# cg-tuwien/ppsurf

Measured on AMD Instinct MI355X. Metric: occupancy query-points/sec @ res=257, 50NN, higher is better.
Workload: dtype f16x3

## Files before the change

### ppsurf_amd/csrc/pps_decode.hip

```cpp
#include <cstdlib>
#include "pps_common.h"
#include "../../include/ppsurf_amd.h"

using namespace pps;

#ifndef NT
#define NT 256
#endif
#define NW (NT / 64)
#ifndef WG_PER_CU
#define WG_PER_CU (512 / NT)
#endif
#ifndef PPS_PRIO
#define PPS_PRIO 1
#endif
#ifndef PPS_PRIO_PN
#define PPS_PRIO_PN 1
#endif
#define CH4 2048

template <int CHUNK_F4_NEXT, int NTH = NT, class F>
__device__ __forceinline__ void stream_step(const f32x4* __restrict__ gnext, f32x4*& cur, f32x4*& nxt, F&& compute) {
    chunk_copy_async<CHUNK_F4_NEXT / NTH, NTH>(gnext, nxt);
    compute((const f32x4*)cur);
// ... 579 lines not shown
#pragma unroll
    for (int h = 0; h < PN_C2N; ++h)
        stream_step<PCH4, PNT>(wg + 2048 + (h + 1) * PCH4, cur, nxt, [&](const f32x4* w) {
            dense_blocks_f16x3<2, PN_C2OB, 1>(a, (const half8*)w, bias4 + 48 + 4 * PN_C2OB * h, lane,
                                              [&](int i, const f32x4& o0, const f32x4& o1) { y[PN_C2OB / 2 * h + i] = split_f16_r(amax, o0, o1); }); });
#pragma unroll
    for (int c = 0; c < PN_C3N - 1; ++c)
        stream_step<PCH4, PNT>(wg + 4096 + (c + 1) * PCH4, cur, nxt, [&](const f32x4* w) {
            dense_blocks_f16x3<4, PN_C3OB, 1>(y, (const half8*)w, bias4 + 80 + 4 * PN_C3OB * c, lane,
                                              [&](int i, const f32x4& o0, const f32x4& o1) { z[PN_C3OB * c + 2 * i] = o0; z[PN_C3OB * c + 2 * i + 1] = o1; }); });
    stream_step<1024, PNT>(wg, cur, nxt, [&](const f32x4* w) {
        dense_blocks_f16x3<4, PN_C3OB, 1>(y, (const half8*)w, bias4 + 80 + 4 * PN_C3OB * (PN_C3N - 1), lane,
                                          [&](int i, const f32x4& o0, const f32x4& o1) { z[PN_C3OB * (PN_C3N - 1) + 2 * i] = o0; z[PN_C3OB * (PN_C3N - 1) + 2 * i + 1] = o1; }); });
    __builtin_amdgcn_s_setprio(0);
}

template <int T, class ZSink>
__device__ __forceinline__ void stn_chain_h_tiles(const float (&coord)[T], const float* xyz_l, const f32x4* bias4, const f32x4* wg,
                                                  f32x4*& cur, f32x4*& nxt, int lane, float& amax, ZSink&& zsink) {
    const int g = lane >> 4;
    HiLo a[T][2], b[T][2], y[T][4];
#pragma unroll
    for (int t = 0; t < T; ++t) {
        f32x4 x0[4];
#pragma unroll
        for (int bb = 0; bb < 4; ++bb) x0[bb] = bias4[4 * bb + g];
        xyz_blocks<4>(coord[t], x0, xyz_l, lane);
        relu_blocks<4>(x0);
        a[t][0] = split_f16_r(amax, x0[0], x0[1]);
        a[t][1] = split_f16_r(amax, x0[2], x0[3]);
    }
    __builtin_amdgcn_s_setprio(PPS_PRIO_PN);
    stream_step<1024, PNT>(wg + 1024, cur, nxt, [&](const f32x4* w) {
        dense_blocks_f16x3_tiles<T, 2, 4, 1>(a, (const half8*)w, bias4 + 16, lane, [&](int t, int i, const f32x4& o0, const f32x4& o1) { b[t][i] = split_f16_r(amax, o0, o1); }); });
    stream_step<PCH4, PNT>(wg + 2048, cur, nxt, [&](const f32x4* w) {
        dense_blocks_f16x3_tiles<T, 2, 4, 1>(b, (const half8*)w, bias4 + 32, lane, [&](int t, int i, const f32x4& o0, const f32x4& o1) { a[t][i] = split_f16_r(amax, o0, o1); }); });
#pragma unroll
    for (int h = 0; h < PN_C2N; ++h)
        stream_step<PCH4, PNT>(wg + 2048 + (h + 1) * PCH4, cur, nxt, [&](const f32x4* w) {
            dense_blocks_f16x3_tiles<T, 2, PN_C2OB, 1>(a, (const half8*)w, bias4 + 48 + 4 * PN_C2OB * h, lane,
                                                      [&](int t, int i, const f32x4& o0, const f32x4& o1) { y[t][PN_C2OB / 2 * h + i] = split_f16_r(amax, o0, o1); }); });
#pragma unroll
    for (int c = 0; c < PN_C3N - 1; ++c)
        stream_step<PCH4, PNT>(wg + 4096 + (c + 1) * PCH4, cur, nxt, [&](const f32x4* w) {
            dense_blocks_f16x3_tiles<T, 4, PN_C3OB, 1>(y, (const half8*)w, bias4 + 80 + 4 * PN_C3OB * c, lane,
                                                      [&](int t, int i, const f32x4& o0, const f32x4& o1) { zsink(t, PN_C3OB * c + 2 * i, o0, o1); }); });
    stream_step<1024, PNT>(wg, cur, nxt, [&](const f32x4* w) {
        dense_blocks_f16x3_tiles<T, 4, PN_C3OB, 1>(y, (const half8*)w, bias4 + 80 + 4 * PN_C3OB * (PN_C3N - 1), lane,
                                                  [&](int t, int i, const f32x4& o0, const f32x4& o1) { zsink(t, PN_C3OB * (PN_C3N - 1) + 2 * i, o0, o1); }); });
    __builtin_amdgcn_s_setprio(0);
}

template <bool H>
__global__ __launch_bounds__(PNT, 2) void pointnet_stn_rows_kernel(const float* __restrict__ patches, int64_t Q, int P, int pack,
                                                                   const float* __restrict__ wpack, const f32x4* __restrict__ wdense,
                                                                   const float* __restrict__ bias, float* __restrict__ gout, int* __restrict__ flag) {
    if (!H && gate_closed(flag)) return;
    float amax = 0.f;
    f32x4* buf0 = (f32x4*)pps_smem;
    f32x4* buf1 = buf0 + PCH4;
    float* xyz_l = (float*)(buf1 + PCH4);
    float* bias_l = xyz_l + PA_W_XYZ;
    float* park = bias_l + PA_NBIAS;
    const f32x4* bias4 = (const f32x4*)bias_l;
    const f32x4* wg = wdense;
    const int lane = lane_id(), wave = threadIdx.x >> 6, n = lane & 15, g = lane >> 4;
    float* mypark = park + wave * PN_PARK_ROWS * PN_ROWF;

    lds_fill(xyz_l, wpack, PA_W_XYZ);
    lds_fill(bias_l, bias, PA_NBIAS);
    stream_prologue<1024, PNT>(wg, buf0);
    stream_wait();
    __syncthreads();
    f32x4 *cur = buf0, *nxt = buf1;

    const PatchPacking pk = patch_packing(P, pack);
    const int64_t ngroups = (Q + pk.qg - 1) / pk.qg;
    const int ntiles = (int)((ngroups + PNW - 1) / PNW);
    int first, count, stride;
    xcd_tile_range(ntiles, first, count, stride);
    for (int it = 0; it < count; ++it) {
        const int64_t q0 = ((int64_t)(first + it * stride) * PNW + wave) * pk.qg;
        if constexpr (H) {
            if (pk.packed) {
                const int ql = n / pk.lo;
                const int64_t qq = (q0 + ql < Q) ? q0 + ql : Q - 1;
                const float coord[1] = {(g < 3) ? patches[(qq * P + pk.fb * 16 + (n % pk.lo)) * 3 + g] : 0.f};
                stn_chain_h_tiles<1>(coord, xyz_l, bias4, wg, cur, nxt, lane, amax, [&](int, int bb, const f32x4& o0, const f32x4& o1) {
                    f32x4 m0, m1;
#pragma unroll
                    for (int r = 0; r < 4; ++r) { m0[r] = group_max(o0[r], pk.lo); m1[r] = group_max(o1[r], pk.lo); }
                    if ((n % pk.lo) == 0) { ((f32x4*)(mypark + ql * PN_ROWF))[4 * bb + g] = m0; ((f32x4*)(mypark + ql * PN_ROWF))[4 * (bb + 1) + g] = m1; }
                });
            }
            for (int qi = 0; qi < pk.qg; ++qi) {
                const int64_t q = q0 + qi;
                const bool qv = q < Q;
                const int64_t qc = qv ? q : Q - 1;
                f32x4 rmax[16];
#pragma unroll
                for (int bb = 0; bb < 16; ++bb)
                    rmax[bb] = pk.packed ? ((const f32x4*)(mypark + qi * PN_ROWF))[4 * bb + g] : f32x4{-INFINITY, -INFINITY, -INFINITY, -INFINITY};
                auto zmax = [&](int, int bb, const f32x4& o0, const f32x4& o1) {
#pragma unroll
                    for (int r = 0; r < 4; ++r) { rmax[bb][r] = max_raw(rmax[bb][r], o0[r]); rmax[bb + 1][r] = max_raw(rmax[bb + 1][r], o1[r]); }
                };
                auto row_coord = [&](int rb) {
                    const int row = rb * 16 + n;
                    const int rowc = row < P ? row : P - 1;
                    return (g < 3) ? patches[(qc * P + rowc) * 3 + g] : 0.f;
                };
                int rb = 0;
                for (; rb + 1 < pk.fb; rb += 2) {
                    const float coord[2] = {row_coord(rb), row_coord(rb + 1)};
                    stn_chain_h_tiles<2>(coord, xyz_l, bias4, wg, cur, nxt, lane, amax, zmax);
                }
                if (rb < pk.fb) {
                    const float coord[1] = {row_coord(rb)};
                    stn_chain_h_tiles<1>(coord, xyz_l, bias4, wg, cur, nxt, lane, amax, zmax);
                }
#pragma unroll
                for (int bb = 0; bb < 16; ++bb) {
                    float p0 = rmax[bb][0], p1 = rmax[bb][1], p2 = rmax[bb][2], p3 = rmax[bb][3];
                    row16_max4(p0, p1, p2, p3);
                    if (n == 0 && qv) ((f32x4*)(gout + q * 256))[4 * bb + g] = f32x4{p0, p1, p2, p3};
                }
            }
            continue;
        }
        f32x4 z[16];
        if (pk.packed) {
            const int ql = n / pk.lo;
            const int64_t qq = (q0 + ql < Q) ? q0 + ql : Q - 1;
            const float coord = (g < 3) ? patches[(qq * P + pk.fb * 16 + (n % pk.lo)) * 3 + g] : 0.f;
            if (H) stn_chain_h(coord, z, xyz_l, bias4, wg, cur, nxt, lane, amax); else stn_chain(coord, z, xyz_l, bias4, wg, cur, nxt, lane);
#pragma unroll
            for (int bb = 0; bb < 16; ++bb) {
                f32x4 m;
#pragma unroll
                for (int r = 0; r < 4; ++r) m[r] = group_max(z[bb][r], pk.lo);
                if ((n % pk.lo) == 0) ((f32x4*)(mypark + ql * PN_ROWF))[4 * bb + g] = m;
            }
        }
        for (int qi = 0; qi < pk.qg; ++qi) {
            const int64_t q = q0 + qi;
            const bool qv = q < Q;
            const int64_t qc = qv ? q : Q - 1;
            f32x4 rmax[16];
#pragma unroll
            for (int bb = 0; bb < 16; ++bb)
                rmax[bb] = pk.packed ? ((const f32x4*)(mypark + qi * PN_ROWF))[4 * bb + g] : f32x4{-INFINITY, -INFINITY, -INFINITY, -INFINITY};
            for (int rb = 0; rb < pk.fb; ++rb) {
                const int row = rb * 16 + n;
                const int rowc = row < P ? row : P - 1;
                const float coord = (g < 3) ? patches[(qc * P + rowc) * 3 + g] : 0.f;
                if (H) stn_chain_h(coord, z, xyz_l, bias4, wg, cur, nxt, lane, amax); else stn_chain(coord, z, xyz_l, bias4, wg, cur, nxt, lane);
#pragma unroll
                for (int bb = 0; bb < 16; ++bb)
#pragma unroll
                    for (int r = 0; r < 4; ++r) rmax[bb][r] = max_raw(rmax[bb][r], z[bb][r]);
            }
#pragma unroll
            for (int bb = 0; bb < 16; ++bb) {
                float p0 = rmax[bb][0], p1 = rmax[bb][1], p2 = rmax[bb][2], p3 = rmax[bb][3];
                row16_max4(p0, p1, p2, p3);
                const f32x4 p = {p0, p1, p2, p3};
                if (n == 0 && qv) ((f32x4*)(gout + q * 256))[4 * bb + g] = p;
            }
        }
    }
    if (H) range_commit(amax, flag);
}

#define PB_NBIAS (128 + 64 + 4096)
#define PB_LDS_BYTES (2 * CH4 * 16 + 4096 * 4)
#ifndef PB_T
#define PB_T 1
#endif

__global__ __launch_bounds__(NT, 2) void pointnet_stn_fc_kernel(const float* __restrict__ gin, int64_t Q,
                                                                const float* __restrict__ wpack, const float* __restrict__ bias,
                                                                float* __restrict__ trans2, const int* __restrict__ gate) {
    if (gate_closed(gate)) return;
    f32x4* buf0 = (f32x4*)pps_smem;
    f32x4* buf1 = buf0 + CH4;
    float* bias_l = (float*)(buf1 + CH4);
    const f32x4* bias4 = (const f32x4*)bias_l;
    const f32x4* wg = (const f32x4*)wpack;
    const int lane = lane_id(), wave = threadIdx.x >> 6, n = lane & 15, g = lane >> 4;

    lds_fill(bias_l, bias + 192, 4096);
    const f32x4* bias_g = (const f32x4*)bias;
    stream_prologue<CH4>(wg, buf0);
    stream_wait();
    __syncthreads();
    f32x4 *cur = buf0, *nxt = buf1;

    const int ntiles = (int)((Q + NW * 16 * PB_T - 1) / (NW * 16 * PB_T));
    int first, count, stride;
    xcd_tile_range(ntiles, first, count, stride);
    for (int it = 0; it < count; ++it) {
        f32x4 u[PB_T][4];
        int64_t qcs[PB_T];
        bool qvs[PB_T];
#pragma unroll
        for (int t = 0; t < PB_T; ++t) {
            const int64_t qi = (int64_t)(first + it * stride) * (NW * 16 * PB_T) + (wave * PB_T + t) * 16 + n;
            qvs[t] = qi < Q;
            qcs[t] = qvs[t] ? qi : Q - 1;
            f32x4 a[16], h[8];
            {
                const f32x4* src = (const f32x4*)(gin + qcs[t] * 256) + g;
#pragma unroll
                for (int bb = 0; bb < 16; ++bb) a[bb] = src[4 * bb];
            }
#pragma unroll
            for (int c = 0; c < 4; ++c)
                stream_step<CH4>(wg + (c + 1) * CH4, cur, nxt,
                               [&](const f32x4* w) { dense_blocks<16, 2, 1>(a, &h[2 * c], w, bias_g + 8 * c, lane); });
            stream_step<CH4>(t + 1 < PB_T ? wg : wg + 5 * CH4, cur, nxt,
                           [&](const f32x4* w) { dense_blocks<8, 4, 1>(h, u[t], w, bias_g + 32, lane); });
        }
#pragma unroll 1
        for (int c = 0; c < 32; ++c) {
            f32x4 o[PB_T][8];
            const f32x4* gn = (c + 1 < 32) ? wg + (6 + c) * CH4 : wg;
            stream_step<CH4>(gn, cur, nxt, [&](const f32x4* w) {
#pragma unroll
                for (int t = 0; t < PB_T; ++t) dense_blocks<4, 8, 0>(u[t], o[t], w, bias4 + 32 * c, lane);
            });
#pragma unroll
            for (int t = 0; t < PB_T; ++t) {
                if (qvs[t]) {
                    f32x4* dst = (f32x4*)(trans2 + qcs[t] * 4096) + g;
#pragma unroll
                    for (int j = 0; j < 8; ++j) dst[4 * (8 * c + j)] = o[t][j];
                }
            }
        }
    }
}

__global__ __launch_bounds__(NT, 2) void pointnet_stn_fc_h_kernel(const float* __restrict__ gin, int64_t Q, const f32x4* __restrict__ w16,
                                                                  const float* __restrict__ bias, half8* __restrict__ trans2h, int* __restrict__ range) {
    float amax = 0.f;
    f32x4* buf0 = (f32x4*)pps_smem;
    f32x4* buf1 = buf0 + CH4;
    float* bias_l = (float*)(buf1 + CH4);
    const f32x4* bias4 = (const f32x4*)bias_l;
    const f32x4* wg = w16;
    const int lane = lane_id(), wave = threadIdx.x >> 6, n = lane & 15, g = lane >> 4;

    lds_fill(bias_l, bias + 192, 4096);
    const f32x4* bias_g = (const f32x4*)bias;
    stream_prologue<CH4>(wg, buf0);
    stream_wait();
    __syncthreads();
    f32x4 *cur = buf0, *nxt = buf1;
    const int ntiles = (int)((Q + NW * 16 - 1) / (NW * 16));
    int first, count, stride;
    xcd_tile_range(ntiles, first, count, stride);
    for (int it = 0; it < count; ++it) {
        const int64_t qi = (int64_t)(first + it * stride) * (NW * 16) + wave * 16 + n;
        const bool qv = qi < Q;
        const int64_t qc = qv ? qi : Q - 1;
        HiLo ah[8], h[4], u[2];
        {
            f32x4 a[16];
            const f32x4* src = (const f32x4*)(gin + qc * 256) + g;
#pragma unroll
            for (int bb = 0; bb < 16; ++bb) a[bb] = src[4 * bb];
#pragma unroll
            for (int kb = 0; kb < 8; ++kb) ah[kb] = split_f16_r(amax, a[2 * kb], a[2 * kb + 1]);
        }
#pragma unroll
        for (int c = 0; c < 4; ++c)
            stream_step<CH4>(wg + (c + 1) * CH4, cur, nxt, [&](const f32x4* w) {
                dense_blocks_f16x3<8, 2, 1>(ah, (const half8*)w, bias_g + 8 * c, lane, [&](int, const f32x4& o0, const f32x4& o1) { h[c] = split_f16_r(amax, o0, o1); }); });
        stream_step<CH4>(wg + 5 * CH4, cur, nxt, [&](const f32x4* w) {
            dense_blocks_f16x3<4, 4, 1>(h, (const half8*)w, bias_g + 32, lane, [&](int i, const f32x4& o0, const f32x4& o1) { u[i] = split_f16_r(amax, o0, o1); }); });
        half8* dst = trans2h + qc * 1024 + g;
#pragma unroll 1
        for (int c = 0; c < 32; ++c) {
            const f32x4* gn = (c + 1 < 32) ? wg + (6 + c) * CH4 : wg;
            stream_step<CH4>(gn, cur, nxt, [&](const f32x4* w) {
                dense_blocks_f16x3<2, 8, 0, false>(u, (const half8*)w, bias4 + 32 * c, lane, [&](int i, const f32x4& o0, const f32x4& o1) {
                    const int a = 2 * c + (i >> 1), kb = i & 1;
                    const HiLo v = split_f16_r(amax, o0, o1);
                    if (qv) {
                        half8* d = dst + (((a >> 4) * 2 + kb) * 2) * 64 + 4 * (a & 15);
                        d[0] = v.hi;
                        d[64] = v.lo;
                    }
                }); });
        }
    }
    range_commit(amax, range);
}

#define PC_W_XYZ 256
#define PC_NBIAS (576 + 256 + 4)
#define PC_WFLOATS (4096 + 8192)
#define PC_LDS_BYTES ((PC_WFLOATS + PC_W_XYZ + PC_NBIAS) * 4)

template <bool H>
__global__ __launch_bounds__(PNT, 2) void pointnet_feat_rows_kernel(const float* __restrict__ patches, const float* __restrict__ trans2,
                                                                    int64_t Q, int P, const float* __restrict__ wpack,
                                                                    const f32x4* __restrict__ wdense, const float* __restrict__ bias,
                                                                    float* __restrict__ xbar, int* __restrict__ flag) {
    if (!H && gate_closed(flag)) return;
    float amax = 0.f;
    f32x4* w_l = (f32x4*)pps_smem;
    float* xyz_l = (float*)(w_l + PC_WFLOATS / 4);
    float* bias_l = xyz_l + PC_W_XYZ;
    const f32x4* bias4 = (const f32x4*)bias_l;
    const f32x4* u4 = bias4 + 144;
    const int lane = lane_id(), wave = threadIdx.x >> 6, n = lane & 15, g = lane >> 4;
    for (int i = threadIdx.x; i < PC_WFLOATS / 4; i += PNT) w_l[i] = wdense[i];
    lds_fill(xyz_l, wpack, PC_W_XYZ);
    lds_fill(bias_l, bias, PC_NBIAS);
    __syncthreads();
    const float s0 = bias_l[576 + 256];
    const f32x4* w_c0b = w_l;
    const f32x4* w_c2 = w_l + 1024;
    const int ntile_rows = (P + 15) / 16;

    const int ntiles = (int)((Q + PNW - 1) / PNW);
    int first, count, stride;
    xcd_tile_range(ntiles, first, count, stride);
    for (int it = 0; it < count; ++it) {
        const int64_t q = (int64_t)(first + it * stride) * PNW + wave;
        if (q >= Q) continue;
        half8 th[4][2], tl[4][2];
        f32x4 tf[4][4];
        if (H) {
            const half8* tq = (const half8*)trans2 + q * 1024 + 4 * n + g;
#pragma unroll
            for (int ob = 0; ob < 4; ++ob)
#pragma unroll
                for (int kb = 0; kb < 2; ++kb) { th[ob][kb] = tq[((ob * 2 + kb) * 2) * 64]; tl[ob][kb] = tq[((ob * 2 + kb) * 2 + 1) * 64]; }
        } else {
            const f32x4* tq = (const f32x4*)(trans2 + q * 4096);
#pragma unroll
            for (int ob = 0; ob < 4; ++ob)
#pragma unroll
                for (int kb = 0; kb < 4; ++kb) tf[ob][kb] = tq[(16 * ob + n) * 16 + 4 * kb + g];
        }
        f32x4 acc[8];
        float mrun = -INFINITY, ssum = 0.f;
#pragma unroll
        for (int bb = 0; bb < 8; ++bb) acc[bb] = f32x4{0.f, 0.f, 0.f, 0.f};
        for (int rb = 0; rb < ntile_rows; ++rb) {
            const int rowi = rb * 16 + n;
            const bool valid = rowi < P;
            const int rowc = valid ? rowi : P - 1;
            const float coord = (g < 3) ? patches[(q * P + rowc) * 3 + g] : 0.f;
            f32x4 x0[4], y[8];
#pragma unroll
            for (int bb = 0; bb < 4; ++bb) x0[bb] = bias4[4 * bb + g];
            xyz_blocks<4>(coord, x0, xyz_l, lane);
            relu_blocks<4>(x0);
            __builtin_amdgcn_s_setprio(PPS_PRIO_PN);
            float s = 0.f;
            if (H) {
                HiLo a[2], b[2];
                a[0] = split_f16_r(amax, x0[0], x0[1]);
                a[1] = split_f16_r(amax, x0[2], x0[3]);
                dense_blocks_f16x3<2, 4, 1>(a, (const half8*)w_c0b, bias4 + 16, lane, [&](int i, const f32x4& o0, const f32x4& o1) { b[i] = split_f16_r(amax, o0, o1); });
#pragma unroll
                for (int ob = 0; ob < 4; ++ob) {
                    f32x4 o = bias4[32 + 4 * ob + g], c = {0.f, 0.f, 0.f, 0.f};
#pragma unroll
                    for (int kb = 0; kb < 2; ++kb) {
                        o = __builtin_amdgcn_mfma_f32_16x16x32_f16(th[ob][kb], b[kb].hi, o, 0, 0, 0);
                        c = __builtin_amdgcn_mfma_f32_16x16x32_f16(th[ob][kb], b[kb].lo, c, 0, 0, 0);
                        c = __builtin_amdgcn_mfma_f32_16x16x32_f16(tl[ob][kb], b[kb].hi, c, 0, 0, 0);
                    }
                    o += c;
#pragma unroll
                    for (int r = 0; r < 4; ++r) x0[ob][r] = fmaxf(o[r], 0.f);
                }
                a[0] = split_f16_r(amax, x0[0], x0[1]);
                a[1] = split_f16_r(amax, x0[2], x0[3]);
                dense_blocks_f16x3<2, 8, 1>(a, (const half8*)w_c2, bias4 + 48, lane, [&](int i, const f32x4& o0, const f32x4& o1) {
                    const f32x4 w0 = u4[4 * (2 * i) + g], w1 = u4[4 * (2 * i + 1) + g];
#pragma unroll
                    for (int r = 0; r < 4; ++r) s += w0[r] * o0[r] + w1[r] * o1[r];
                    y[2 * i] = o0;
                    y[2 * i + 1] = o1;
                });
            } else {
                f32x4 x1[4];
                dense_blocks<4, 4, 1>(x0, x1, w_c0b, bias4 + 16, lane);
#pragma unroll
                for (int ob = 0; ob < 4; ++ob) {
                    f32x4 o = bias4[32 + 4 * ob + g];
#pragma unroll
                    for (int kb = 0; kb < 4; ++kb) {
                        o = __builtin_amdgcn_mfma_f32_16x16x4f32(tf[ob][kb].x, x1[kb].x, o, 0, 0, 0);
                        o = __builtin_amdgcn_mfma_f32_16x16x4f32(tf[ob][kb].y, x1[kb].y, o, 0, 0, 0);
                        o = __builtin_amdgcn_mfma_f32_16x16x4f32(tf[ob][kb].z, x1[kb].z, o, 0, 0, 0);
                        o = __builtin_amdgcn_mfma_f32_16x16x4f32(tf[ob][kb].w, x1[kb].w, o, 0, 0, 0);
                    }
#pragma unroll
                    for (int r = 0; r < 4; ++r) x0[ob][r] = fmaxf(o[r], 0.f);
                }
                dense_blocks<4, 8, 1>(x0, y, w_c2, bias4 + 48, lane);
#pragma unroll
                for (int bb = 0; bb < 8; ++bb) {
                    const f32x4 w4 = u4[4 * bb + g];
#pragma unroll
                    for (int r = 0; r < 4; ++r) s += w4[r] * y[bb][r];
                }
            }
            __builtin_amdgcn_s_setprio(0);
            s += __shfl_xor(s, 16);
            s += __shfl_xor(s, 32);
            s += s0;
            const float mblk = row16_max(valid ? s : -INFINITY);
            const float mnew = fmaxf(mrun, mblk);
            const float scale = __expf(mrun - mnew);
            const float en = valid ? __expf(s - mnew) : 0.f;
            mrun = mnew;
            ssum = ssum * scale + en;
#pragma unroll
            for (int bb = 0; bb < 8; ++bb)
#pragma unroll
                for (int r = 0; r < 4; ++r) acc[bb][r] = acc[bb][r] * scale + en * y[bb][r];
        }
        const float inv = 1.f / row16_sum(ssum);
        rows16_sum_transposed8(acc, lane);
        if (n < 8) ((f32x4*)(xbar + q * 128))[4 * n + g] = acc[0] * inv;
    }
    if (H) range_commit(amax, flag);
}

#define TL_NBIAS (256 + 256 + 32)
#define TL_LDS_BYTES (2 * CH4 * 16 + TL_NBIAS * 4)

__global__ __launch_bounds__(NT, 2) void decode_tail_kernel(const float* __restrict__ pooled, const float* __restrict__ xbar, int64_t Q,
                                                            const float* __restrict__ wpack, const float* __restrict__ bias,
                                                            float* __restrict__ logits, float* __restrict__ occ, int* __restrict__ gate) {
    if (gate_closed(gate)) return;
    if (gate != nullptr && blockIdx.x == 0 && threadIdx.x == 0) atomicAdd(gate + 1, 1);
    f32x4* buf0 = (f32x4*)pps_smem;
    f32x4* buf1 = buf0 + CH4;
    float* bias_l = (float*)(buf1 + CH4);
    const f32x4* bias4 = (const f32x4*)bias_l;
    const f32x4* wg = (const f32x4*)wpack;
    const int lane = lane_id(), wave = threadIdx.x >> 6, n = lane & 15, g = lane >> 4;

    lds_fill(bias_l, bias, TL_NBIAS);
    stream_prologue<CH4>(wg, buf0);
    stream_wait();
    __syncthreads();
    f32x4 *cur = buf0, *nxt = buf1;

    const int ntiles = (int)((Q + NW * 16 - 1) / (NW * 16));
    int first, count, stride;
    xcd_tile_range(ntiles, first, count, stride);
    for (int it = 0; it < count; ++it) {
        const int64_t qi = (int64_t)(first + it * stride) * (NW * 16) + wave * 16 + n;
        const bool qv = qi < Q;
        const int64_t qc = qv ? qi : Q - 1;
        f32x4 p[16], x[8], h[16];
        {
            const f32x4* sp = (const f32x4*)(pooled + qc * 256) + g;
            const f32x4* sx = (const f32x4*)(xbar + qc * 128) + g;
#pragma unroll
            for (int bb = 0; bb < 16; ++bb) p[bb] = sp[4 * bb];
#pragma unroll
            for (int bb = 0; bb < 8; ++bb) x[bb] = sx[4 * bb];
        }
#pragma unroll
        for (int c = 0; c < 8; ++c)
            stream_step<CH4>(wg + (c + 1) * CH4, cur, nxt,
                           [&](const f32x4* w) { dense_blocks<16, 2, 0>(p, &h[2 * c], w, bias4 + 8 * c, lane); });
#pragma unroll
        for (int c = 0; c < 4; ++c)
            stream_step<CH4>(wg + (c + 9) * CH4, cur, nxt,
                           [&](const f32x4* w) { dense_blocks<8, 4, 1, 1>(x, &h[4 * c], w, bias4, lane); });
#pragma unroll
        for (int c = 0; c < 8; ++c)
            stream_step<CH4>(wg + (c + 13) * CH4, cur, nxt,
                           [&](const f32x4* w) { dense_blocks<16, 2, 1>(h, &p[2 * c], w, bias4 + 64 + 8 * c, lane); });
        f32x4 o[2];
        stream_step<CH4>(wg, cur, nxt, [&](const f32x4* w) { dense_blocks<16, 2, 0>(p, o, w, bias4 + 128, lane); });
        if (qv && g == 0) {
            const float l0 = o[0].x, l1 = o[0].y;
            logits[qi * 2] = l0;
            logits[qi * 2 + 1] = l1;
            if (occ) {
                const float mx = fmaxf(l0, l1);
                const float e0 = __expf(l0 - mx), e1 = __expf(l1 - mx);
                occ[qi] = (e0 - e1) / (e0 + e1);
            }
        }
    }
}

__global__ __launch_bounds__(NT, 2) void decode_tail_h_kernel(const float* __restrict__ pooled, const float* __restrict__ xbar, int64_t Q,
                                                              const f32x4* __restrict__ w16, const float* __restrict__ bias,
                                                              float* __restrict__ logits, float* __restrict__ occ, int* __restrict__ range) {
    float amax = 0.f;
    f32x4* buf0 = (f32x4*)pps_smem;
    f32x4* buf1 = buf0 + CH4;
    float* bias_l = (float*)(buf1 + CH4);
    const f32x4* bias4 = (const f32x4*)bias_l;
    const f32x4* wg = w16;
    const int lane = lane_id(), wave = threadIdx.x >> 6, n = lane & 15, g = lane >> 4;

// ... 6 lines not shown
    const int ntiles = (int)((Q + NW * 16 - 1) / (NW * 16));
    int first, count, stride;
    xcd_tile_range(ntiles, first, count, stride);
    for (int it = 0; it < count; ++it) {
        const int64_t qi = (int64_t)(first + it * stride) * (NW * 16) + wave * 16 + n;
        const bool qv = qi < Q;
        const int64_t qc = qv ? qi : Q - 1;
        HiLo p[8], x[4];
        {
            const f32x4* sp = (const f32x4*)(pooled + qc * 256) + g;
            const f32x4* sx = (const f32x4*)(xbar + qc * 128) + g;
#pragma unroll
            for (int kb = 0; kb < 8; ++kb) p[kb] = split_f16_r(amax, sp[4 * (2 * kb)], sp[4 * (2 * kb + 1)]);
#pragma unroll
            for (int kb = 0; kb < 4; ++kb) x[kb] = split_f16_r(amax, sx[4 * (2 * kb)], sx[4 * (2 * kb + 1)]);
        }
        HiLo y[8];
#pragma unroll
        for (int c = 0; c < 8; ++c) {
            f32x4 h[2];
            stream_step<CH4 / 2>(wg + c * 3072 + 2048, cur, nxt, [&](const f32x4* w) {
                dense_blocks_f16x3<8, 2, 0>(p, (const half8*)w, bias4 + 8 * c, lane, [&](int, const f32x4& o0, const f32x4& o1) { h[0] = o0; h[1] = o1; }); });
            stream_step<CH4>(c + 1 < 8 ? wg + (c + 1) * 3072 : wg + 24576, cur, nxt, [&](const f32x4* w) {
                dense_blocks_f16x3<4, 2, 1, true, true>(x, (const half8*)w, bias4, lane, [&](int, const f32x4& o0, const f32x4& o1) { y[c] = split_f16_r(amax, o0, o1); }, h); });
        }
#pragma unroll
        for (int c = 0; c < 8; ++c)
            stream_step<CH4>(wg + 24576 + (c + 1) * 2048, cur, nxt, [&](const f32x4* w) {
                dense_blocks_f16x3<8, 2, 1>(y, (const half8*)w, bias4 + 64 + 8 * c, lane, [&](int, const f32x4& o0, const f32x4& o1) { p[c] = split_f16_r(amax, o0, o1); }); });
        f32x4 o[2];
        stream_step<CH4>(wg, cur, nxt, [&](const f32x4* w) {
            dense_blocks_f16x3<8, 2, 0>(p, (const half8*)w, bias4 + 128, lane, [&](int, const f32x4& o0, const f32x4& o1) { o[0] = o0; o[1] = o1; }); });
        if (qv && g == 0) {
            const float l0 = o[0].x, l1 = o[0].y;
            logits[qi * 2] = l0;
            logits[qi * 2 + 1] = l1;
            if (occ) {
                const float mx = fmaxf(l0, l1);
                const float e0 = __expf(l0 - mx), e1 = __expf(l1 - mx);
                occ[qi] = (e0 - e1) / (e0 + e1);
            }
        }
    }
    range_commit(amax, range);
}

static int g_cu_count = 0;
static int cu_count() {
    if (g_cu_count == 0) {
        int dev = 0;
        hipDeviceProp_t prop;
        if (hipGetDevice(&dev) != hipSuccess || hipGetDeviceProperties(&prop, dev) != hipSuccess) return -1;
        g_cu_count = prop.multiProcessorCount;
    }
    return g_cu_count;
}

template <class K>
static int set_lds(K kernel, int bytes) {
    return hipFuncSetAttribute((const void*)kernel, hipFuncAttributeMaxDynamicSharedMemorySize, bytes) == hipSuccess ? 0 : 1;
}

static int grid_for(int64_t ntiles) {
    int cus = cu_count();
    if (cus <= 0) cus = 256;
    cus *= WG_PER_CU;
    return (int)(ntiles < cus ? (ntiles > 0 ? ntiles : 1) : cus);
}

struct PnSplit { int64_t q_packed; int grid_packed, grid_rest, rest_mode; };
static PnSplit pn_split(int64_t q, int p) {
    int cus = cu_count();
    if (cus <= 0) cus = 256;
    const PatchPacking pk = patch_packing(p);
    PnSplit sp;
    const int wgs = cus * PN_WG_PER_CU;
    const int64_t per_round = (int64_t)wgs * PNW * pk.qg;
    sp.q_packed = pk.packed ? (q / per_round) * per_round : 0;
    if (pk.packed && getenv("PPS_PN_FORCE_PACK")) sp.q_packed = q;
    sp.grid_packed = wgs;
    sp.rest_mode = pk.packed ? 2 : 0;
    const int64_t rest_tiles = (q - sp.q_packed + PNW - 1) / PNW;
    sp.grid_rest = (int)(rest_tiles < wgs ? rest_tiles : wgs);
    return sp;
}

#define PPS_LAUNCH_CHECK() (hipGetLastError() == hipSuccess ? PPS_OK : PPS_ERR_LAUNCH)

template <bool H>
static int launch_stn_rows(const float* patches, int64_t q, int p, const float* wpack, const void* wdense, const float* bias, float* g,
                           int* flag, void* stream) {
    static int once = set_lds(pointnet_stn_rows_kernel<H>, PA_LDS_BYTES);
    (void)once;
    const PnSplit sp = pn_split(q, p);
    if (sp.q_packed > 0)
        hipLaunchKernelGGL(pointnet_stn_rows_kernel<H>, dim3(sp.grid_packed), dim3(PNT), PA_LDS_BYTES, (hipStream_t)stream, patches,
                           sp.q_packed, p, 1, wpack, (const f32x4*)wdense, bias, g, flag);
    if (q > sp.q_packed)
        hipLaunchKernelGGL(pointnet_stn_rows_kernel<H>, dim3(sp.grid_rest), dim3(PNT), PA_LDS_BYTES, (hipStream_t)stream,
                           patches + sp.q_packed * p * 3, q - sp.q_packed, p, sp.rest_mode, wpack, (const f32x4*)wdense, bias, g + sp.q_packed * 256, flag);
    return PPS_LAUNCH_CHECK();
}

template <bool H>
static int launch_feat_rows(const float* patches, const float* trans2, int64_t q, int p, const float* wpack, const void* wdense,
                            const float* bias, float* xbar, int* flag, void* stream) {
    static int once = set_lds(pointnet_feat_rows_kernel<H>, PC_LDS_BYTES);
    (void)once;
    int cus = cu_count();
    if (cus <= 0) cus = 256;
    const int64_t ntiles = (q + PNW - 1) / PNW, wgs = (int64_t)cus * PN_WG_PER_CU;
    hipLaunchKernelGGL(pointnet_feat_rows_kernel<H>, dim3((unsigned)(ntiles < wgs ? ntiles : wgs)), dim3(PNT), PC_LDS_BYTES, (hipStream_t)stream, patches,
                       trans2, q, p, wpack, (const f32x4*)wdense, bias, xbar, flag);
    return PPS_LAUNCH_CHECK();
}


static int interp_pool_f32_impl(const float* G, const float* pts, const float* query, const int64_t* idx, int64_t q, int k,
                                const float* wpack, const float* bias, float* pooled, const int* gate, void* stream) {
    if (q < 0 || k < 1 || k > 64) return PPS_ERR_ARG;
    if (q == 0) return PPS_OK;
    if (!G || !pts || !query || !idx || !wpack || !bias || !pooled) return PPS_ERR_ARG;
    static int once = set_lds(interp_pool_kernel, IP_LDS_BYTES);
    (void)once;
    hipLaunchKernelGGL(interp_pool_kernel, dim3(grid_for((q + NW / 4 - 1) / (NW / 4))), dim3(NT), IP_LDS_BYTES, (hipStream_t)stream,
                       G, pts, query, idx, q, k, wpack, bias, pooled, gate);
    return PPS_LAUNCH_CHECK();
}

static int stn_fc_f32_impl(const float* g, int64_t q, const float* wpack, const float* bias, float* trans2, const int* gate, void* stream) {
    if (q < 0) return PPS_ERR_ARG;
    if (q == 0) return PPS_OK;
    if (!g || !wpack || !bias || !trans2) return PPS_ERR_ARG;
    static int once = set_lds(pointnet_stn_fc_kernel, PB_LDS_BYTES);
    (void)once;
    hipLaunchKernelGGL(pointnet_stn_fc_kernel, dim3(grid_for((q + NW * 16 * PB_T - 1) / (NW * 16 * PB_T))), dim3(NT), PB_LDS_BYTES, (hipStream_t)stream,
                       g, q, wpack, bias, trans2, gate);
    return PPS_LAUNCH_CHECK();
}

static int decode_tail_f32_impl(const float* pooled, const float* xbar, int64_t q, const float* wpack, const float* bias,
                                float* logits, float* occ, int* gate, void* stream) {
    if (q < 0) return PPS_ERR_ARG;
    if (q == 0) return PPS_OK;
    if (!pooled || !xbar || !wpack || !bias || !logits) return PPS_ERR_ARG;
    static int once = set_lds(decode_tail_kernel, TL_LDS_BYTES);
    (void)once;
    hipLaunchKernelGGL(decode_tail_kernel, dim3(grid_for((q + NW * 16 - 1) / (NW * 16))), dim3(NT), TL_LDS_BYTES, (hipStream_t)stream,
                       pooled, xbar, q, wpack, bias, logits, occ, gate);
    return PPS_LAUNCH_CHECK();
}

extern "C" {

int pps_abi_version(void) { return 2; }

int pps_debug_occupancy(int which) {
    int n = -1;
    if (which == 0) { set_lds(interp_pool_kernel, IP_LDS_BYTES); hipOccupancyMaxActiveBlocksPerMultiprocessor(&n, interp_pool_kernel, NT, IP_LDS_BYTES); }
    if (which == 1) { set_lds(pointnet_stn_rows_kernel<false>, PA_LDS_BYTES); hipOccupancyMaxActiveBlocksPerMultiprocessor(&n, pointnet_stn_rows_kernel<false>, PNT, PA_LDS_BYTES); }
    if (which == 3) { set_lds(pointnet_stn_fc_kernel, PB_LDS_BYTES); hipOccupancyMaxActiveBlocksPerMultiprocessor(&n, pointnet_stn_fc_kernel, NT, PB_LDS_BYTES); }
    if (which == 4) { set_lds(pointnet_stn_fc_h_kernel, PB_LDS_BYTES); hipOccupancyMaxActiveBlocksPerMultiprocessor(&n, pointnet_stn_fc_h_kernel, NT, PB_LDS_BYTES); }
    if (which == 2) { set_lds(pointnet_feat_rows_kernel<false>, PC_LDS_BYTES); hipOccupancyMaxActiveBlocksPerMultiprocessor(&n, pointnet_feat_rows_kernel<false>, PNT, PC_LDS_BYTES); }
    return n;
}
int pps_device_cu_count(void) { return cu_count(); }
// ... 27 lines not shown
    if (cus <= 0) cus = 256;
    const int64_t ntiles = (q + IH_NW / 4 - 1) / (IH_NW / 4);
    const int64_t wgs = (int64_t)cus * IH_WG_PER_CU;
    const int grid = (int)(ntiles < wgs ? ntiles : wgs);
    hipLaunchKernelGGL(interp_pool_f16x3_kernel, dim3(grid), dim3(IH_NT), IH_LDS_BYTES, (hipStream_t)stream,
                       G, pts, query, idx, q, k, wxyz, (const f32x4*)w16, bias, pooled, (int*)range_flag);
    return PPS_LAUNCH_CHECK();
}

int pps_interp_small_f32(const float* G, const float* pts, const float* query, const int64_t* idx, int64_t q, int k, int c,
                         const float* wpack, const float* bias, const float* wtail, int nout, float* out, void* stream) {
    if (q < 0 || k < 1 || k > 64 || (c != 32 && c != 64) || nout < 1 || nout > IS_MAX_OUT) return PPS_ERR_ARG;
    if (q == 0) return PPS_OK;
    if (!G || !pts || !query || !idx || !wpack || !bias || !wtail || !out) return PPS_ERR_ARG;
    int cus = cu_count();
    if (cus <= 0) cus = 256;
    const int grid = (int)(q < (int64_t)cus * 8 ? q : (int64_t)cus * 8);
    hipStream_t st = (hipStream_t)stream;
    if (c == 32) hipLaunchKernelGGL((interp_small_kernel<2, false>), dim3(grid), dim3(IS_NT), 0, st, G, pts, query, idx, q, k, wpack, nullptr, bias, wtail, nout, out, nullptr);
    else hipLaunchKernelGGL((interp_small_kernel<4, false>), dim3(grid), dim3(IS_NT), 0, st, G, pts, query, idx, q, k, wpack, nullptr, bias, wtail, nout, out, nullptr);
    return PPS_LAUNCH_CHECK();
}

int pps_interp_small_f16x3(const float* G, const float* pts, const float* query, const int64_t* idx, int64_t q, int k, int c,
                           const float* wpack, const void* w16, const float* bias, const float* wtail, int nout, float* out, int* guard,
                           void* stream) {
    if (q < 0 || k < 1 || k > 64 || (c != 32 && c != 64) || nout < 1 || nout > IS_MAX_OUT) return PPS_ERR_ARG;
    if (q == 0) return PPS_OK;
    if (!G || !pts || !query || !idx || !wpack || !w16 || !bias || !wtail || !out || !guard) return PPS_ERR_ARG;
    int cus = cu_count();
    if (cus <= 0) cus = 256;
    const int grid = (int)(q < (int64_t)cus * 8 ? q : (int64_t)cus * 8);
    hipStream_t st = (hipStream_t)stream;
    if (hipMemsetAsync(guard, 0, sizeof(int), st) != hipSuccess) return PPS_ERR_LAUNCH;
    const float* wh = (const float*)w16;
    if (c == 32) {
        hipLaunchKernelGGL((interp_small_kernel<2, true>), dim3(grid), dim3(IS_NT), 0, st, G, pts, query, idx, q, k, wpack, wh, bias, wtail, nout, out, guard);
        hipLaunchKernelGGL((interp_small_kernel<2, false>), dim3(grid), dim3(IS_NT), 0, st, G, pts, query, idx, q, k, wpack, nullptr, bias, wtail, nout, out, guard);
    } else {
        hipLaunchKernelGGL((interp_small_kernel<4, true>), dim3(grid), dim3(IS_NT), 0, st, G, pts, query, idx, q, k, wpack, wh, bias, wtail, nout, out, guard);
        hipLaunchKernelGGL((interp_small_kernel<4, false>), dim3(grid), dim3(IS_NT), 0, st, G, pts, query, idx, q, k, wpack, nullptr, bias, wtail, nout, out, guard);
    }
    return PPS_LAUNCH_CHECK();
}

int pps_pointnet_stn_rows_f32(const float* patches, int64_t q, int p, const float* wpack, const float* bias, float* g,
                              void* stream) {
    if (q < 0 || p < 1) return PPS_ERR_ARG;
    if (q == 0) return PPS_OK;
    if (!patches || !wpack || !bias || !g) return PPS_ERR_ARG;
    return launch_stn_rows<false>(patches, q, p, wpack, wpack + PA_W_XYZ, bias, g, nullptr, stream);
}

int pps_pointnet_stn_fc_f32(const float* g, int64_t q, const float* wpack, const float* bias, float* trans2, void* stream) {
    return stn_fc_f32_impl(g, q, wpack, bias, trans2, nullptr, stream);
}

int pps_pointnet_feat_rows_f32(const float* patches, const float* trans2, int64_t q, int p, const float* wpack,
                               const float* bias, float* xbar, void* stream) {
    if (q < 0 || p < 1) return PPS_ERR_ARG;
    if (q == 0) return PPS_OK;
    if (!patches || !trans2 || !wpack || !bias || !xbar) return PPS_ERR_ARG;
    return launch_feat_rows<false>(patches, trans2, q, p, wpack, wpack + PC_W_XYZ, bias, xbar, nullptr, stream);
}

int pps_pointnet_f16x3(const float* patches, int64_t q, int p, const float* const* weights ,
                       const void* const* w16, float* g, float* trans2, float* xbar, int32_t* range_flag, void* const* events, void* stream) {
    if (q < 0 || p < 1) return PPS_ERR_ARG;
    if (q == 0) return PPS_OK;
    if (!patches || !weights || !w16 || !w16[0] || !w16[1] || !w16[2] || !g || !trans2 || !xbar) return PPS_ERR_ARG;
    hipStream_t st = (hipStream_t)stream;
    int* range = (int*)range_flag;
    int rc = launch_stn_rows<true>(patches, q, p, weights[0], w16[0], weights[1], g, range, stream);
    if (events && events[0]) hipEventRecord((hipEvent_t)events[0], st);
    if (rc != PPS_OK) return rc;
    static int once = set_lds(pointnet_stn_fc_h_kernel, PB_LDS_BYTES);
    (void)once;
    static const int64_t sub = getenv("PPS_PN_SUB") ? atoll(getenv("PPS_PN_SUB")) : 0;
    static const bool reuse = getenv("PPS_PN_SUB_REUSE") != nullptr;
    if (sub > 0 && sub < q) {
        for (int64_t off = 0; off < q && rc == PPS_OK; off += sub) {
            const int64_t n = q - off < sub ? q - off : sub;
            float* t2 = reuse ? trans2 : trans2 + off * 4096;
            hipLaunchKernelGGL(pointnet_stn_fc_h_kernel, dim3(grid_for((n + NW * 16 - 1) / (NW * 16))), dim3(NT), PB_LDS_BYTES, st, g + off * 256, n,
                               (const f32x4*)w16[1], weights[3], (half8*)t2, range);
            rc = launch_feat_rows<true>(patches + off * p * 3, t2, n, p, weights[4], w16[2], weights[5], xbar + off * 128, range, stream);
        }
        if (events && events[1]) hipEventRecord((hipEvent_t)events[1], st);
        if (events && events[2]) hipEventRecord((hipEvent_t)events[2], st);
        return rc;
    }
    hipLaunchKernelGGL(pointnet_stn_fc_h_kernel, dim3(grid_for((q + NW * 16 - 1) / (NW * 16))), dim3(NT), PB_LDS_BYTES, st, g, q,
                       (const f32x4*)w16[1], weights[3], (half8*)trans2, range);
    if (events && events[1]) hipEventRecord((hipEvent_t)events[1], st);
    if (hipGetLastError() != hipSuccess) return PPS_ERR_LAUNCH;
    rc = launch_feat_rows<true>(patches, trans2, q, p, weights[4], w16[2], weights[5], xbar, range, stream);
    if (events && events[2]) hipEventRecord((hipEvent_t)events[2], st);
    return rc;
}

int pps_decode_tail_f32(const float* pooled, const float* xbar, int64_t q, const float* wpack, const float* bias,
                        float* logits, float* occ, void* stream) {
    return decode_tail_f32_impl(pooled, xbar, q, wpack, bias, logits, occ, nullptr, stream);
}

int pps_decode_tail_f16x3(const float* pooled, const float* xbar, int64_t q, const void* w16, const float* bias, float* logits, float* occ,
                          int32_t* range_flag, void* stream) {
    if (q < 0) return PPS_ERR_ARG;
    if (q == 0) return PPS_OK;
    if (!pooled || !xbar || !w16 || !bias || !logits) return PPS_ERR_ARG;
    static int once = set_lds(decode_tail_h_kernel, TL_LDS_BYTES);
    (void)once;
    hipLaunchKernelGGL(decode_tail_h_kernel, dim3(grid_for((q + NW * 16 - 1) / (NW * 16))), dim3(NT), TL_LDS_BYTES, (hipStream_t)stream,
                       pooled, xbar, q, (const f32x4*)w16, bias, logits, occ, (int*)range_flag);
    return PPS_LAUNCH_CHECK();
}

#define PPS_DECODE_WS_HEAD 64
size_t pps_decode_ws_bytes(int64_t q) { return q < 0 ? 0 : (size_t)q * (256 + 256 + 4096 + 256) * sizeof(float) + PPS_DECODE_WS_HEAD; }

static int decode_fwd(const float* table, const float* pts, const float* query, const int64_t* idx, int64_t q, int k,
                      const float* patches, int p, const float* const* weights, float* logits, float* occ, void* ws, void* const* events,
                      void* stream, const void* const* w16 = nullptr) {
    const void* interp_w16 = w16 ? w16[0] : nullptr;
    const bool pn16 = w16 && w16[1] && w16[2] && w16[3];
    if (q < 0) return PPS_ERR_ARG;
    if (q == 0) return PPS_OK;
    if (!weights || !ws || !logits) return PPS_ERR_ARG;
    for (int i = 0; i < 10; ++i)
        if (!weights[i]) return PPS_ERR_ARG;
    int* guard = (int*)ws;
    float* pooled = (float*)ws + PPS_DECODE_WS_HEAD / sizeof(float);
    float* g = pooled + q * 256;
    float* trans2 = g + q * 256;
    float* xbar = trans2 + q * 4096;
    hipStream_t st = (hipStream_t)stream;
    const bool split = interp_w16 || pn16 || (w16 && w16[4]);
    if (split && hipMemsetAsync(guard, 0, sizeof(int), st) != hipSuccess) return PPS_ERR_LAUNCH;
#define PPS_MARK(i) do { if (events && events[i] && hipEventRecord((hipEvent_t)events[i], st) != hipSuccess) return PPS_ERR_LAUNCH; } while (0)
    PPS_MARK(0);
    int rc = interp_w16 ? pps_interp_pool_f16x3(table, pts, query, idx, q, k, weights[0], interp_w16, weights[1], pooled, guard, stream)
                        : pps_interp_pool_f32(table, pts, query, idx, q, k, weights[0], weights[1], pooled, stream);
    PPS_MARK(1);
    if (pn16) {
        if (rc == PPS_OK) rc = pps_pointnet_f16x3(patches, q, p, weights + 2, w16 + 1, g, trans2, xbar, guard, events ? events + 2 : nullptr, stream);
    } else {
        if (rc == PPS_OK) rc = pps_pointnet_stn_rows_f32(patches, q, p, weights[2], weights[3], g, stream);
        PPS_MARK(2);
        if (rc == PPS_OK) rc = pps_pointnet_stn_fc_f32(g, q, weights[4], weights[5], trans2, stream);
        PPS_MARK(3);
        if (rc == PPS_OK) rc = pps_pointnet_feat_rows_f32(patches, trans2, q, p, weights[6], weights[7], xbar, stream);
        PPS_MARK(4);
    }
    if (rc == PPS_OK)
        rc = (w16 && w16[4]) ? pps_decode_tail_f16x3(pooled, xbar, q, w16[4], weights[9], logits, occ, guard, stream)
                             : pps_decode_tail_f32(pooled, xbar, q, weights[8], weights[9], logits, occ, stream);
    PPS_MARK(5);
#undef PPS_MARK
    if (split && rc == PPS_OK) {
        rc = interp_pool_f32_impl(table, pts, query, idx, q, k, weights[0], weights[1], pooled, guard, stream);
        if (rc == PPS_OK) rc = launch_stn_rows<false>(patches, q, p, weights[2], weights[2] + PA_W_XYZ, weights[3], g, guard, stream);
        if (rc == PPS_OK) rc = stn_fc_f32_impl(g, q, weights[4], weights[5], trans2, guard, stream);
        if (rc == PPS_OK) rc = launch_feat_rows<false>(patches, trans2, q, p, weights[6], weights[6] + PC_W_XYZ, weights[7], xbar, guard, stream);
        if (rc == PPS_OK) rc = decode_tail_f32_impl(pooled, xbar, q, weights[8], weights[9], logits, occ, guard, stream);
    }
    return rc;
}

int pps_decode_fwd_f32(const float* table, const float* pts, const float* query, const int64_t* idx, int64_t q, int k,
                       const float* patches, int p, const float* const* weights, float* logits, float* occ, void* ws, void* stream) {
    return decode_fwd(table, pts, query, idx, q, k, patches, p, weights, logits, occ, ws, nullptr, stream);
}

int pps_decode_fwd_events_f32(const float* table, const float* pts, const float* query, const int64_t* idx, int64_t q, int k,
                              const float* patches, int p, const float* const* weights, float* logits, float* occ, void* ws,
// ... 13 lines not shown
```

Baseline: 12.57 million.

## Pair odd leftover tiles, balance FC waves, DPP-merge stores, prefetch trans2, skip rescale

Several independent changes land in the pointnet path. In the STN rows kernel, when a row-tile count is odd, leftover tiles from adjacent queries are paired into two-tile chain calls so fewer single-tile passes run. The FC kernel takes a variable queries-per-wave count chosen on the host to balance the final round across CUs, and it merges pairs of outputs across lanes with DPP before issuing contiguous nontemporal stores. The feature kernel prefetches the next query's trans2 matrix during the last tile, and the online-softmax rescale is skipped when the running max is unchanged. Together these add complexity, a wave-uniform branch, and extra register pressure from the prefetched buffers.

```diff
diff --git a/ppsurf_amd/csrc/pps_decode.hip b/ppsurf_amd/csrc/pps_decode.hip
--- a/ppsurf_amd/csrc/pps_decode.hip
+++ b/ppsurf_amd/csrc/pps_decode.hip
@@ -685,7 +685,14 @@
     for (int it = 0; it < count; ++it) {
         const int64_t q0 = ((int64_t)(first + it * stride) * PNW + wave) * pk.qg;
         if constexpr (H) {
-            if (pk.packed) {
+            const bool odd = pk.packed && (pk.fb & 1);
+            const bool left_in_regs = odd && pk.qg == 1;
+            auto row_coord = [&](int64_t qc, int rb) {
+                const int row = rb * 16 + n;
+                const int rowc = row < P ? row : P - 1;
+                return (g < 3) ? patches[(qc * P + rowc) * 3 + g] : 0.f;
+            };
+            if (pk.packed && !left_in_regs) {
                 const int ql = n / pk.lo;
                 const int64_t qq = (q0 + ql < Q) ? q0 + ql : Q - 1;
                 const float coord[1] = {(g < 3) ? patches[(qq * P + pk.fb * 16 + (n % pk.lo)) * 3 + g] : 0.f};
@@ -700,26 +707,43 @@
                 const int64_t q = q0 + qi;
                 const bool qv = q < Q;
                 const int64_t qc = qv ? q : Q - 1;
+                if (odd && !left_in_regs && (qi & 1) == 0) {
+                    const int64_t qn = (q + 1 < Q) ? q + 1 : Q - 1;
+                    const float coord[2] = {row_coord(qc, pk.fb - 1), row_coord(qn, pk.fb - 1)};
+                    stn_chain_h_tiles<2>(coord, xyz_l, bias4, wg, cur, nxt, lane, amax, [&](int t, int bb, const f32x4& o0, const f32x4& o1) {
+#pragma unroll
+                        for (int j = 0; j < 2; ++j) {
+                            const f32x4& o = j ? o1 : o0;
+                            float a0 = o[0], a1 = o[1], a2 = o[2], a3 = o[3];
+                            row16_max4(a0, a1, a2, a3);
+                            f32x4* d = (f32x4*)(mypark + (qi + t) * PN_ROWF) + 4 * (bb + j) + g;
+                            if (n == 0) {
+                                const f32x4 p = *d;
+                                *d = f32x4{max_raw(p[0], a0), max_raw(p[1], a1), max_raw(p[2], a2), max_raw(p[3], a3)};
+                            }
+                        }
+                    });
+                }
                 f32x4 rmax[16];
 #pragma unroll
                 for (int bb = 0; bb < 16; ++bb)
-                    rmax[bb] = pk.packed ? ((const f32x4*)(mypark + qi * PN_ROWF))[4 * bb + g] : f32x4{-INFINITY, -INFINITY, -INFINITY, -INFINITY};
+                    rmax[bb] = pk.packed && !left_in_regs ? ((const f32x4*)(mypark + qi * PN_ROWF))[4 * bb + g] : f32x4{-INFINITY, -INFINITY, -INFINITY, -INFINITY};
                 auto zmax = [&](int, int bb, const f32x4& o0, const f32x4& o1) {
 #pragma unroll
                     for (int r = 0; r < 4; ++r) { rmax[bb][r] = max_raw(rmax[bb][r], o0[r]); rmax[bb + 1][r] = max_raw(rmax[bb + 1][r], o1[r]); }
                 };
-                auto row_coord = [&](int rb) {
-                    const int row = rb * 16 + n;
-                    const int rowc = row < P ? row : P - 1;
-                    return (g < 3) ? patches[(qc * P + rowc) * 3 + g] : 0.f;
-                };
-                int rb = 0;
-                for (; rb + 1 < pk.fb; rb += 2) {
-                    const float coord[2] = {row_coord(rb), row_coord(rb + 1)};
+                const int fb_own = odd ? pk.fb - 1 : pk.fb;
+                if (left_in_regs) {
+                    const float coord[2] = {(g < 3) ? patches[(qc * P + pk.fb * 16 + (n % pk.lo)) * 3 + g] : 0.f, row_coord(qc, pk.fb - 1)};
                     stn_chain_h_tiles<2>(coord, xyz_l, bias4, wg, cur, nxt, lane, amax, zmax);
                 }
-                if (rb < pk.fb) {
-                    const float coord[1] = {row_coord(rb)};
+                int rb = 0;
+                for (; rb + 1 < fb_own; rb += 2) {
+                    const float coord[2] = {row_coord(qc, rb), row_coord(qc, rb + 1)};
+                    stn_chain_h_tiles<2>(coord, xyz_l, bias4, wg, cur, nxt, lane, amax, zmax);
+                }
+                if (rb < fb_own) {
+                    const float coord[1] = {row_coord(qc, rb)};
                     stn_chain_h_tiles<1>(coord, xyz_l, bias4, wg, cur, nxt, lane, amax, zmax);
                 }
 #pragma unroll
@@ -777,6 +801,10 @@
 
 #define PB_NBIAS (128 + 64 + 4096)
 #define PB_LDS_BYTES (2 * CH4 * 16 + 4096 * 4)
+#ifndef PPS_FC_NT
+#define PPS_FC_NT 1
+#endif
+
 #ifndef PB_T
 #define PB_T 1
 #endif
@@ -844,7 +872,7 @@
     }
 }
 
-__global__ __launch_bounds__(NT, 2) void pointnet_stn_fc_h_kernel(const float* __restrict__ gin, int64_t Q, const f32x4* __restrict__ w16,
+__global__ __launch_bounds__(NT, 2) void pointnet_stn_fc_h_kernel(const float* __restrict__ gin, int64_t Q, int VQ, const f32x4* __restrict__ w16,
                                                                   const float* __restrict__ bias, half8* __restrict__ trans2h, int* __restrict__ range) {
     float amax = 0.f;
     f32x4* buf0 = (f32x4*)pps_smem;
@@ -860,13 +888,13 @@
     stream_wait();
     __syncthreads();
     f32x4 *cur = buf0, *nxt = buf1;
-    const int ntiles = (int)((Q + NW * 16 - 1) / (NW * 16));
+    const int ntiles = (int)((Q + NW * VQ - 1) / (NW * VQ));
     int first, count, stride;
     xcd_tile_range(ntiles, first, count, stride);
     for (int it = 0; it < count; ++it) {
-        const int64_t qi = (int64_t)(first + it * stride) * (NW * 16) + wave * 16 + n;
-        const bool qv = qi < Q;
-        const int64_t qc = qv ? qi : Q - 1;
+        const int64_t qi = (int64_t)(first + it * stride) * (NW * VQ) + wave * VQ + n;
+        const bool qv = n < VQ && qi < Q;
+        const int64_t qc = qv ? qi : (qi - n < Q ? qi - n : Q - 1);
         HiLo ah[8], h[4], u[2];
         {
             f32x4 a[16];
@@ -882,18 +910,38 @@
                 dense_blocks_f16x3<8, 2, 1>(ah, (const half8*)w, bias_g + 8 * c, lane, [&](int, const f32x4& o0, const f32x4& o1) { h[c] = split_f16_r(amax, o0, o1); }); });
         stream_step<CH4>(wg + 5 * CH4, cur, nxt, [&](const f32x4* w) {
             dense_blocks_f16x3<4, 4, 1>(h, (const half8*)w, bias_g + 32, lane, [&](int i, const f32x4& o0, const f32x4& o1) { u[i] = split_f16_r(amax, o0, o1); }); });
-        half8* dst = trans2h + qc * 1024 + g;
+        const int64_t tq0 = qi - n;
+        const bool upper = n >= 8;
+        const bool qva = (n & 7) < VQ && tq0 + (n & 7) < Q, qvb = (n | 8) < VQ && tq0 + (n | 8) < Q;
+        half8* dsta = trans2h + (qva ? tq0 + (n & 7) : 0) * 1024 + g + 4 * (n >> 3);
+        half8* dstb = trans2h + (qvb ? tq0 + (n | 8) : 0) * 1024 + g + 4 * (n >> 3);
 #pragma unroll 1
         for (int c = 0; c < 32; ++c) {
             const f32x4* gn = (c + 1 < 32) ? wg + (6 + c) * CH4 : wg;
+            HiLo even[2];
             stream_step<CH4>(gn, cur, nxt, [&](const f32x4* w) {
                 dense_blocks_f16x3<2, 8, 0, false>(u, (const half8*)w, bias4 + 32 * c, lane, [&](int i, const f32x4& o0, const f32x4& o1) {
-                    const int a = 2 * c + (i >> 1), kb = i & 1;
+                    const int kb = i & 1;
                     const HiLo v = split_f16_r(amax, o0, o1);
-                    if (qv) {
-                        half8* d = dst + (((a >> 4) * 2 + kb) * 2) * 64 + 4 * (a & 15);
-                        d[0] = v.hi;
-                        d[64] = v.lo;
+                    if (i < 2) { even[kb] = v; return; }
+                    const int off = ((((2 * c) >> 4) * 2 + kb) * 2) * 64 + 4 * ((2 * c) & 15);
+#pragma unroll
+                    for (int part = 0; part < 2; ++part) {
+                        const u32x4 r0 = __builtin_bit_cast(u32x4, part ? even[kb].lo : even[kb].hi), r1 = __builtin_bit_cast(u32x4, part ? v.lo : v.hi);
+                        u32x4 xa, xb;
+#pragma unroll
+                        for (int d = 0; d < 4; ++d) {
+                            const unsigned r = (unsigned)__builtin_amdgcn_update_dpp(0, (int)(upper ? r0[d] : r1[d]), 0x128, 0xf, 0xf, false);
+                            xa[d] = upper ? r : r0[d];
+                            xb[d] = upper ? r1[d] : r;
+                        }
+#if PPS_FC_NT
+                        if (qva) __builtin_nontemporal_store(__builtin_bit_cast(half8, xa), dsta + off + part * 64);
+                        if (qvb) __builtin_nontemporal_store(__builtin_bit_cast(half8, xb), dstb + off + part * 64);
+#else
+                        if (qva) dsta[off + part * 64] = __builtin_bit_cast(half8, xa);
+                        if (qvb) dstb[off + part * 64] = __builtin_bit_cast(half8, xb);
+#endif
                     }
                 }); });
         }
@@ -931,24 +979,29 @@
     const int ntiles = (int)((Q + PNW - 1) / PNW);
     int first, count, stride;
     xcd_tile_range(ntiles, first, count, stride);
+    half8 th[4][2], tl[4][2];
+    f32x4 tf[4][4];
+    auto load_m = [&](int64_t qm) {
+        if (H) {
+            const half8* tq = (const half8*)trans2 + qm * 1024 + 4 * n + g;
+#pragma unroll
+            for (int ob = 0; ob < 4; ++ob)
+#pragma unroll
+                for (int kb = 0; kb < 2; ++kb) { th[ob][kb] = tq[((ob * 2 + kb) * 2) * 64]; tl[ob][kb] = tq[((ob * 2 + kb) * 2 + 1) * 64]; }
+        } else {
+            const f32x4* tq = (const f32x4*)(trans2 + qm * 4096);
+#pragma unroll
+            for (int ob = 0; ob < 4; ++ob)
+#pragma unroll
+                for (int kb = 0; kb < 4; ++kb) tf[ob][kb] = tq[(16 * ob + n) * 16 + 4 * kb + g];
+        }
+    };
+    if (count > 0 && (int64_t)first * PNW + wave < Q) load_m((int64_t)first * PNW + wave);
     for (int it = 0; it < count; ++it) {
         const int64_t q = (int64_t)(first + it * stride) * PNW + wave;
-        if (q >= Q) continue;
-        half8 th[4][2], tl[4][2];
-        f32x4 tf[4][4];
-        if (H) {
-            const half8* tq = (const half8*)trans2 + q * 1024 + 4 * n + g;
-#pragma unroll
-            for (int ob = 0; ob < 4; ++ob)
-#pragma unroll
-                for (int kb = 0; kb < 2; ++kb) { th[ob][kb] = tq[((ob * 2 + kb) * 2) * 64]; tl[ob][kb] = tq[((ob * 2 + kb) * 2 + 1) * 64]; }
-        } else {
-            const f32x4* tq = (const f32x4*)(trans2 + q * 4096);
-#pragma unroll
-            for (int ob = 0; ob < 4; ++ob)
-#pragma unroll
-                for (int kb = 0; kb < 4; ++kb) tf[ob][kb] = tq[(16 * ob + n) * 16 + 4 * kb + g];
-        }
+        if (q >= Q) break;
+        const int64_t qnext = q + (int64_t)stride * PNW;
+        const bool prefetch = it + 1 < count && qnext < Q;
         f32x4 acc[8];
         float mrun = -INFINITY, ssum = 0.f;
 #pragma unroll
@@ -983,6 +1036,7 @@
 #pragma unroll
                     for (int r = 0; r < 4; ++r) x0[ob][r] = fmaxf(o[r], 0.f);
                 }
+                if (rb + 1 == ntile_rows && prefetch) load_m(qnext);
                 a[0] = split_f16_r(amax, x0[0], x0[1]);
                 a[1] = split_f16_r(amax, x0[2], x0[3]);
                 dense_blocks_f16x3<2, 8, 1>(a, (const half8*)w_c2, bias4 + 48, lane, [&](int i, const f32x4& o0, const f32x4& o1) {
@@ -1008,6 +1062,7 @@
 #pragma unroll
                     for (int r = 0; r < 4; ++r) x0[ob][r] = fmaxf(o[r], 0.f);
                 }
+                if (rb + 1 == ntile_rows && prefetch) load_m(qnext);
                 dense_blocks<4, 8, 1>(x0, y, w_c2, bias4 + 48, lane);
 #pragma unroll
                 for (int bb = 0; bb < 8; ++bb) {
@@ -1022,14 +1077,21 @@
             s += s0;
             const float mblk = row16_max(valid ? s : -INFINITY);
             const float mnew = fmaxf(mrun, mblk);
-            const float scale = __expf(mrun - mnew);
             const float en = valid ? __expf(s - mnew) : 0.f;
-            mrun = mnew;
-            ssum = ssum * scale + en;
+            if (__builtin_amdgcn_readfirstlane((int)(mnew != mrun))) {
+                const float scale = __expf(mrun - mnew);
+                mrun = mnew;
+                ssum = ssum * scale;
+#pragma unroll
+                for (int bb = 0; bb < 8; ++bb)
+#pragma unroll
+                    for (int r = 0; r < 4; ++r) acc[bb][r] = acc[bb][r] * scale;
+            }
+            ssum = ssum + en;
 #pragma unroll
             for (int bb = 0; bb < 8; ++bb)
 #pragma unroll
-                for (int r = 0; r < 4; ++r) acc[bb][r] = acc[bb][r] * scale + en * y[bb][r];
+                for (int r = 0; r < 4; ++r) acc[bb][r] = acc[bb][r] + en * y[bb][r];
         }
         const float inv = 1.f / row16_sum(ssum);
         rows16_sum_transposed8(acc, lane);
@@ -1202,6 +1264,21 @@
     sp.rest_mode = pk.packed ? 2 : 0;
     const int64_t rest_tiles = (q - sp.q_packed + PNW - 1) / PNW;
     sp.grid_rest = (int)(rest_tiles < wgs ? rest_tiles : wgs);
+    return sp;
+}
+
+struct PnFcSplit { int vq, grid; };
+static PnFcSplit pn_fc_split(int64_t q) {
+    int cus = cu_count();
+    if (cus <= 0) cus = 256;
+    const int64_t wgs = (int64_t)cus * WG_PER_CU;
+    const int64_t rounds = ((q + NW * 16 - 1) / (NW * 16) + wgs - 1) / wgs;
+    PnFcSplit sp;
+    sp.vq = rounds > 1 ? (int)((q + wgs * NW * rounds - 1) / (wgs * NW * rounds)) : 16;
+    if (sp.vq < 1) sp.vq = 1;
+    if (sp.vq > 16) sp.vq = 16;
+    const int64_t ntiles = (q + NW * sp.vq - 1) / (NW * sp.vq);
+    sp.grid = (int)(ntiles < wgs ? (ntiles > 0 ? ntiles : 1) : wgs);
     return sp;
 }
 
@@ -1395,7 +1472,8 @@
         for (int64_t off = 0; off < q && rc == PPS_OK; off += sub) {
             const int64_t n = q - off < sub ? q - off : sub;
             float* t2 = reuse ? trans2 : trans2 + off * 4096;
-            hipLaunchKernelGGL(pointnet_stn_fc_h_kernel, dim3(grid_for((n + NW * 16 - 1) / (NW * 16))), dim3(NT), PB_LDS_BYTES, st, g + off * 256, n,
+            const PnFcSplit fs = pn_fc_split(n);
+            hipLaunchKernelGGL(pointnet_stn_fc_h_kernel, dim3(fs.grid), dim3(NT), PB_LDS_BYTES, st, g + off * 256, n, fs.vq,
                                (const f32x4*)w16[1], weights[3], (half8*)t2, range);
             rc = launch_feat_rows<true>(patches + off * p * 3, t2, n, p, weights[4], w16[2], weights[5], xbar + off * 128, range, stream);
         }
@@ -1403,7 +1481,8 @@
         if (events && events[2]) hipEventRecord((hipEvent_t)events[2], st);
         return rc;
     }
-    hipLaunchKernelGGL(pointnet_stn_fc_h_kernel, dim3(grid_for((q + NW * 16 - 1) / (NW * 16))), dim3(NT), PB_LDS_BYTES, st, g, q,
+    const PnFcSplit fs = pn_fc_split(q);
+    hipLaunchKernelGGL(pointnet_stn_fc_h_kernel, dim3(fs.grid), dim3(NT), PB_LDS_BYTES, st, g, q, fs.vq,
                        (const f32x4*)w16[1], weights[3], (half8*)trans2, range);
     if (events && events[1]) hipEventRecord((hipEvent_t)events[1], st);
     if (hipGetLastError() != hipSuccess) return PPS_ERR_LAUNCH;
```

Result: no change. 12.69 million (median of 6 runs) (+0.9%).
